# mjhoptics/ray-optics

Measured on AMD Instinct MI355X. Metric: ray-surface intersections/sec, higher is better.
Workload: dtype f64; 1 GPU; double-Gauss 13 interfaces (K=12), 1 field, 1 wvl, 1024x1024 pupil grid per GPU, FULL ray packets, device-generated rays (BASELINE.json configs[1]); interfaces=13, out_mode=FULL, field_index=0

## Files before the change

include/roxtrace.h:

```cpp
#ifndef ROXTRACE_H
#define ROXTRACE_H

#include <stddef.h>
#include <stdint.h>

#ifdef __cplusplus
extern "C" {
#endif
#if defined(__GNUC__) || defined(__clang__)
#pragma GCC visibility push(default)
#endif

#define ROX_ABI_VERSION 8
#define ROX_MAX_COEF 10
#define ROX_MAX_AP 4
#define ROX_SEG_DOUBLES 10

enum { ROX_TRANSMIT = 0, ROX_REFLECT = 1, ROX_DUMMY = 2, ROX_PHANTOM = 3 };
enum { ROX_SPHERICAL = 0, ROX_CONIC = 1, ROX_EVENPOLY = 2, ROX_RADIALPOLY = 3,
       ROX_YTOROID = 4, ROX_XTOROID = 5, ROX_THINLENS = 6 };
enum { ROX_PH_NONE = 0,
       ROX_PH_GRATING = 1,
       ROX_PH_DOE_RADIAL = 2,
       ROX_PH_HOLOGRAM = 3 };
// ... 90 lines not shown
    double cr_last_d[3];
    double d_cr_b4[3];
    double v_be;
    double image_pt[3];
} rox_wavefront;

typedef struct rox_opts {
    uint32_t flags;
    int32_t out_mode;
    int32_t first_surf;
    int32_t last_surf;
    double eps;
    double fuzz;
    double foc;
    double image_pt[2];
    rox_wavefront wf;
} rox_opts;

enum { ROX_FLD_EPD = 0, ROX_FLD_EPD_WIDE = 1, ROX_FLD_AIM_PT = 2, ROX_FLD_NA = 3,
       ROX_FLD_FNO = 4, ROX_FLD_AIM_DIR = 5 };

typedef struct rox_field {
    double pt0[3];
    double aim[2];
    double eprad;
    double z_enp;
    double vlx, vux, vly, vuy;
    double z_dir0;
    int32_t kind;
    int32_t rot_order;
    double rot[9];
    double cr_dir[2];
} rox_field;

typedef struct rox_grid {
    double start[2];
    double stop[2];
    int32_t num;
    int32_t kind;
    int32_t row_begin;
    int32_t row_count;
} rox_grid;

typedef struct rox_out {
    double *seg;
    double *op;
    uint8_t *status;
    int16_t *fail_surf;
    double *pupil;
    int64_t ld;
    int64_t *n_hits;
} rox_out;

typedef struct rox_system rox_system;

int rox_abi_version(void);
int rox_device_count(int *count);
int rox_set_device(int device);
const char *rox_last_error(void);

int rox_pin_host_memory(void *p, size_t bytes, void **device_ptr);
int rox_unpin_host_memory(void *p);
int rox_copy_async(void *dst, const void *src, size_t bytes, void *stream);
int rox_synchronize(void *stream);

int rox_system_create(const rox_surface *rows, int32_t n_ifcs,
                      const double *n_table, const double *wvls, int32_t n_wvls,
                      rox_system **out_sys);
int rox_system_destroy(rox_system *sys);
int rox_system_num_segments(const rox_system *sys, uint32_t flags,
                            int32_t *n_seg);

typedef struct rox_vig {
    rox_field fld;
    double start_dir[2];
    double unit_dir[2];
    int32_t xy;
    int32_t wvl_idx;
    int32_t stop_surf;
    int32_t max_iter;
} rox_vig;
int rox_calc_vignetting(rox_system *sys, int32_t n, const rox_vig *probs,
                        double eps, double *vig, int32_t *clip_surf, void *stream);

typedef struct rox_pupil_iter {
    rox_field fld;
    double start_r0;
    double r_target;
    int32_t xy;
    int32_t wvl_idx;
    int32_t indx;
    int32_t pad;
} rox_pupil_iter;
int rox_iterate_pupil_rays(rox_system *sys, int32_t n, const rox_pupil_iter *probs,
                           double eps, double *start_r, void *stream);

int rox_calc_psf(const double *opd, int32_t ndim, int32_t maxdim, double *psf,
                 uint32_t flags, void *stream);

int rox_trace_rays(rox_system *sys, int64_t n_rays,
                   const double *pt0, const double *dir0,
                   const int32_t *wvl_idx, int32_t wvl_idx_all,
                   const rox_opts *opts, const rox_out *out, void *stream);

int rox_trace_pupil_grid(rox_system *sys, const rox_field *fld,
                         const rox_grid *grid, int32_t wvl_idx,
// ... 274 lines not shown
```

include/roxtrace_diag.h:

```cpp
#ifndef ROXTRACE_DIAG_H
#define ROXTRACE_DIAG_H

#include "roxtrace.h"

#ifdef __cplusplus
extern "C" {
#endif
#if defined(__GNUC__) || defined(__clang__)
#pragma GCC visibility push(default)
#endif

int rox_time_pupil_grid(rox_system *sys, const rox_field *fld,
                        const rox_grid *grid, int32_t wvl_idx,
                        const rox_opts *opts, const rox_out *out,
                        void *stream, int32_t launches, double *mean_ms);

int rox_selftest_fp64(uint64_t n, uint64_t seed, uint64_t counts[4]);

int rox_diag_pack_launches(uint64_t counts[2]);

#if defined(__GNUC__) || defined(__clang__)
#pragma GCC visibility pop
#endif
#ifdef __cplusplus
}
#endif
#endif
```

ray-optics_amd/abi.py:

```python
import ctypes as C

ABI_VERSION = 8
MAX_COEF = 10
MAX_AP = 4
SEG_DOUBLES = 10

TRANSMIT, REFLECT, DUMMY, PHANTOM = 0, 1, 2, 3
MODE_NAMES = {'transmit': TRANSMIT, 'reflect': REFLECT, 'dummy': DUMMY,
              'phantom': PHANTOM}
SPHERICAL, CONIC, EVENPOLY, RADIALPOLY, YTOROID, XTOROID, THINLENS = 0, 1, 2, 3, 4, 5, 6
PROFILE_NAMES = {'Spherical': SPHERICAL, 'Conic': CONIC,
                 'EvenPolynomial': EVENPOLY, 'RadialPolynomial': RADIALPOLY,
                 'YToroid': YTOROID, 'XToroid': XTOROID}
PH_NONE, PH_GRATING, PH_DOE_RADIAL, PH_HOLOGRAM = 0, 1, 2, 3
AP_CIRCULAR, AP_RECTANGULAR, AP_ALWAYS_BLOCK = 0, 1, 2
OK, MISSED_SURFACE, TIR, BLOCKED, EVANESCENT = 0, 1, 2, 3, 4
OUT_FULL, OUT_LAST, OUT_HITS, OUT_OPD, OUT_HITS_COMPACT, OUT_FAN = 0, 1, 2, 3, 4, 5
CHECK_APERTURES = 1
INTERSECT_OBJ = 2
FILTER_PHANTOMS = 4
APPLY_VIGNETTING = 8
HOST_POINTERS = 16
HITS_APPEND = 32
FAST_FP64 = 64
# ... 206 lines not shown


WD_SLOT_COLS = 11
MAX_WD_AUX = 32
MAX_WD_COLS = 512


class Vig(C.Structure):
    _fields_ = [('fld', Field), ('start_dir', C.c_double * 2), ('unit_dir', C.c_double * 2),
                ('xy', C.c_int32), ('wvl_idx', C.c_int32), ('stop_surf', C.c_int32),
                ('max_iter', C.c_int32)]


class PupilIter(C.Structure):
    _fields_ = [('fld', Field), ('start_r0', C.c_double), ('r_target', C.c_double),
                ('xy', C.c_int32), ('wvl_idx', C.c_int32), ('indx', C.c_int32), ('pad', C.c_int32)]


assert C.sizeof(Aperture) == 40
assert C.sizeof(Vig) == 240
assert C.sizeof(Phase) == 168
assert C.sizeof(Surface) == 576
assert C.sizeof(Wavefront) == 512
assert C.sizeof(Opts) == 568
assert C.sizeof(Field) == 192
assert C.sizeof(Grid) == 48
assert C.sizeof(Out) == 56
assert C.sizeof(Aim) == 80
assert C.sizeof(Enp) == 136
assert C.sizeof(FocusPlane) == 544
assert C.sizeof(FocusStats) == 72
assert C.sizeof(FocusPsfStats) == 32
assert C.sizeof(ZernikeTerm) == 16
assert C.sizeof(ZernikeStats) == 56
assert C.sizeof(Footprint) == 144
assert C.sizeof(TxSurface) == 64
assert C.sizeof(TxItem) == 72
assert C.sizeof(SaItem) == 144
assert C.sizeof(SegFocus) == 136
assert C.sizeof(WmapItem) == 40
assert C.sizeof(WdItem) == 24

EXPORTS = ('rox_abi_version', 'rox_device_count', 'rox_set_device',
           'rox_last_error', 'rox_system_create', 'rox_system_destroy',
           'rox_system_num_segments', 'rox_trace_rays',
           'rox_trace_pupil_grid', 'rox_trace_pupil_grids', 'rox_trace_pupil_list',
           'rox_aim_chief_rays', 'rox_iterate_ray_raw', 'rox_find_real_enp', 'rox_calc_vignetting',
           'rox_iterate_pupil_rays', 'rox_calc_psf',
           'rox_pin_host_memory', 'rox_unpin_host_memory', 'rox_copy_async', 'rox_synchronize',
           'rox_spot_stats', 'rox_trace_through_focus', 'rox_trace_through_focus_grids',
           'rox_focus_psf', 'rox_focus_mtf', 'rox_focus_ee', 'rox_focus_gmtf', 'rox_focus_psf_ee',
           'rox_focus_zernike', 'rox_surface_footprints', 'rox_surface_transmission',
           'rox_surface_thinfilm', 'rox_projected_solid_angle', 'rox_segment_foci', 'rox_weighted_maps',
           'rox_wave_differentials')
DIAG_EXPORTS = ('rox_time_pupil_grid', 'rox_selftest_fp64', 'rox_diag_pack_launches')


def declare(lib):
    vp, i32, i64, dbl = C.c_void_p, C.c_int32, C.c_int64, C.c_double
    P = C.POINTER
    lib.rox_abi_version.restype = C.c_int
    lib.rox_abi_version.argtypes = []
    lib.rox_device_count.restype = C.c_int
    lib.rox_device_count.argtypes = [P(C.c_int)]
    lib.rox_set_device.restype = C.c_int
    lib.rox_set_device.argtypes = [C.c_int]
    lib.rox_last_error.restype = C.c_char_p
    lib.rox_last_error.argtypes = []
    lib.rox_system_create.restype = C.c_int
    lib.rox_system_create.argtypes = [P(Surface), i32, vp, vp, i32, P(vp)]
    lib.rox_system_destroy.restype = C.c_int
    lib.rox_system_destroy.argtypes = [vp]
    lib.rox_system_num_segments.restype = C.c_int
    lib.rox_system_num_segments.argtypes = [vp, C.c_uint32, P(i32)]
    lib.rox_trace_rays.restype = C.c_int
    lib.rox_trace_rays.argtypes = [vp, i64, vp, vp, vp, i32, P(Opts), P(Out), vp]
    lib.rox_trace_pupil_grid.restype = C.c_int
    lib.rox_trace_pupil_grid.argtypes = [vp, P(Field), P(Grid), i32, P(Opts),
                                         P(Out), vp]
    lib.rox_trace_pupil_grids.restype = C.c_int
    lib.rox_trace_pupil_grids.argtypes = [vp, i32, P(Field), P(i32), P(Grid), P(Opts),
                                          P(Out), vp]
    lib.rox_trace_pupil_list.restype = C.c_int
    lib.rox_trace_pupil_list.argtypes = [vp, P(Field), i64, vp, vp, i32,
                                         P(Opts), P(Out), vp]
    lib.rox_aim_chief_rays.restype = C.c_int
    lib.rox_aim_chief_rays.argtypes = [vp, i32, P(Aim), dbl, vp, vp, vp]
    lib.rox_iterate_ray_raw.restype = C.c_int
    lib.rox_iterate_ray_raw.argtypes = [vp, i32, P(Aim), dbl, vp, vp, vp, vp, vp]
    lib.rox_find_real_enp.restype = C.c_int
    lib.rox_find_real_enp.argtypes = [vp, i32, P(Enp), dbl, vp, vp, vp]
    lib.rox_calc_vignetting.restype = C.c_int
    lib.rox_calc_vignetting.argtypes = [vp, i32, P(Vig), dbl, vp, vp, vp]
    lib.rox_iterate_pupil_rays.restype = C.c_int
    lib.rox_iterate_pupil_rays.argtypes = [vp, i32, P(PupilIter), dbl, vp, vp]
    lib.rox_calc_psf.restype = C.c_int
    lib.rox_calc_psf.argtypes = [vp, i32, i32, vp, C.c_uint32, vp]
    lib.rox_pin_host_memory.restype = C.c_int
    lib.rox_pin_host_memory.argtypes = [vp, C.c_size_t, P(vp)]
    lib.rox_unpin_host_memory.restype = C.c_int
    lib.rox_unpin_host_memory.argtypes = [vp]
    lib.rox_copy_async.restype = C.c_int
    lib.rox_copy_async.argtypes = [vp, vp, C.c_size_t, vp]
    lib.rox_synchronize.restype = C.c_int
    lib.rox_synchronize.argtypes = [vp]
    lib.rox_spot_stats.restype = C.c_int
    lib.rox_spot_stats.argtypes = [vp, i64, vp, vp, i64, i32, vp, i32, vp, i32, P(SpotSummary), vp, vp]
    lib.rox_trace_through_focus.restype = C.c_int
    lib.rox_trace_through_focus.argtypes = [vp, P(Field), P(Grid), i32, P(Opts), i32, P(FocusPlane),
                                            vp, i64, vp, vp, vp]
    lib.rox_trace_through_focus_grids.restype = C.c_int
    lib.rox_trace_through_focus_grids.argtypes = [vp, i32, P(Field), P(i32), P(Grid), P(Opts), i32,
                                                  P(FocusPlane), vp, i64, vp, vp, vp]
    lib.rox_focus_psf.restype = C.c_int
    lib.rox_focus_psf.argtypes = [i32, i32, vp, i64, vp, vp, i32, i32, vp, vp, vp]
    lib.rox_focus_mtf.restype = C.c_int
    lib.rox_focus_mtf.argtypes = [i32, i32, vp, i32, vp, i32, vp, vp, vp]
    lib.rox_focus_ee.restype = C.c_int
    lib.rox_focus_ee.argtypes = [i32, i32, vp, i64, vp, i64, vp, i32, vp, vp, i32, vp, vp, vp, vp]
    lib.rox_focus_gmtf.restype = C.c_int
    lib.rox_focus_gmtf.argtypes = [i32, i32, vp, i64, vp, i64, i32, vp, i32, vp, vp, i32, vp, vp, vp, vp]
    lib.rox_focus_psf_ee.restype = C.c_int
    lib.rox_focus_psf_ee.argtypes = [i32, i32, vp, i32, vp, vp, i32, vp, vp, vp, vp]
    lib.rox_focus_zernike.restype = C.c_int
    lib.rox_focus_zernike.argtypes = [i32, i32, vp, i64, vp, P(Grid), vp, vp, i32, P(ZernikeTerm),
                                      vp, vp, vp]
    lib.rox_surface_footprints.restype = C.c_int
    lib.rox_surface_footprints.argtypes = [vp, C.c_uint32, C.c_uint32, i32, P(Out), i64, vp, vp, i32, vp, vp]
    lib.rox_surface_transmission.restype = C.c_int
    lib.rox_surface_transmission.argtypes = [vp, C.c_uint32, C.c_uint32, i32, P(Out), i64, vp, i32, vp, vp, vp, i64,
                                             vp, vp, vp]
    lib.rox_surface_thinfilm.restype = C.c_int
    lib.rox_surface_thinfilm.argtypes = [vp, C.c_uint32, C.c_uint32, i32, P(Out), i64, vp, vp, i32, vp, vp, vp, vp, vp,
                                         vp, vp, i64, vp, vp, vp]
    lib.rox_projected_solid_angle.restype = C.c_int
    lib.rox_projected_solid_angle.argtypes = [i32, i32, P(Out), i32, vp, i64, vp, vp, vp]
    lib.rox_segment_foci.restype = C.c_int
    lib.rox_segment_foci.argtypes = [vp, C.c_uint32, i32, P(Out), i64, vp, i64, vp, vp, vp]
    lib.rox_weighted_maps.restype = C.c_int
    lib.rox_weighted_maps.argtypes = [vp, C.c_uint32, i32, P(Out), i64, i32, vp, i64, vp, vp, i32, vp, i32, i32, vp, vp,
                                      vp, vp, vp]
    lib.rox_wave_differentials.restype = C.c_int
    lib.rox_wave_differentials.argtypes = [vp, C.c_uint32, i32, P(Out), i64, vp, i32, vp, i32, vp, i64, i64, vp, i64,
                                           vp, vp, vp, vp, vp]
    lib.rox_time_pupil_grid.restype = C.c_int
    lib.rox_time_pupil_grid.argtypes = [vp, P(Field), P(Grid), i32, P(Opts),
                                        P(Out), vp, i32, P(dbl)]
    lib.rox_selftest_fp64.restype = C.c_int
    lib.rox_selftest_fp64.argtypes = [C.c_uint64, C.c_uint64, P(C.c_uint64)]
    lib.rox_diag_pack_launches.restype = C.c_int
    lib.rox_diag_pack_launches.argtypes = [P(C.c_uint64)]
    return lib
```

ray-optics_amd/csrc/launch.hip:

```cpp
#include <atomic>
#include <climits>

#include "rox_system.hpp"
#include "../../include/roxtrace_diag.h"

namespace rox {

bool force_gtab()
{
    static const bool v = env_flag("ROX_FORCE_GTAB");
    return v;
}

static size_t launch_lds(const rox_system *s, int inst, bool per_ray_wvl, bool fast, bool gtab, int out_mode)
{
    const int feat = kInstances[inst];
    const bool phase = gtab || (feat & F_PHASE), aplist = gtab || (feat & F_APLIST);
    const bool global_table = gtab || gtab_of(feat, fast, out_mode) != 0;
    const size_t N = s->n_ifcs, Wn = per_ray_wvl ? (size_t)s->n_wvls : 1;
    size_t b = (global_table ? 0 : N * sizeof(dev_surface)) + Wn * N * sizeof(double) +
               ((phase && !global_table) ? Wn * N * kPhaseConsts * sizeof(double) : 0) +
               ((global_table && aplist) ? N * ROX_MAX_AP * sizeof(double) : 0) +
               ((size_t)s->n_wvls + N) * sizeof(double) + 2 * N * sizeof(int32_t);
    if (fast && !gtab)
// ... 42 lines not shown
        if (!(o->flags & ROX_HITS_APPEND) && out->ld < n_rays)
            return fail(ROX_E_ARG, "HITS_COMPACT: out.ld (%lld pairs of room) < n_rays (%lld)",
                        (long long)out->ld, (long long)n_rays);
        if (out->ld < 0)
            return fail(ROX_E_ARG, "HITS_COMPACT: negative out.ld");
    } else if (out->ld < n_rays) {
        return fail(ROX_E_ARG, "out.ld (%lld) < n_rays (%lld)", (long long)out->ld, (long long)n_rays);
    } else if (o->flags & ROX_HITS_APPEND) {
        return fail(ROX_E_ARG, "ROX_HITS_APPEND goes with ROX_OUT_HITS_COMPACT only");
    }
    if (!out->seg && n_rays > 0)
        return fail(ROX_E_ARG, "out.seg is null");
    if ((o->flags & ROX_FILTER_PHANTOMS) && sys->rows[0].mode == ROX_PHANTOM)
        return fail(ROX_E_UNSUPPORTED, "phantom object surface with filter_out_phantoms");
    return 0;
}

int check_field(const rox_field *fld)
{
    if (!fld)
        return fail(ROX_E_ARG, "null argument");
    if (fld->kind < ROX_FLD_EPD || fld->kind > ROX_FLD_AIM_DIR)
        return fail(ROX_E_ARG, "bad rox_field.kind %d", fld->kind);
    return 0;
}

int blocks_per_cu(int bs)
{
    static const int v = (int)env_int("ROX_BLOCKS_PER_CU", 0);
    return v > 0 ? v : 32 * 256 / bs;
}

int compact_blocks_per_cu()
{
    static const int v = (int)env_int("ROX_COMPACT_BLOCKS_PER_CU", 0);
    return v > 0 ? v : 1;
}

int32_t compact_small_want(const rox_system *sys, int64_t n_rays)
{
    static const int v = (int)env_int("ROX_COMPACT_SMALL_TILES", -1);
    if (v >= 0)
        return v;
    return n_rays <= (int64_t)sys->num_cus * kSmallTile ? sys->num_cus : 0;
}

int64_t rays_per_launch()
{
    static const int64_t v = [] {
        const long long n = env_int("ROX_RAYS_PER_LAUNCH", 0);
        return (n > 0 && n <= (1LL << 28)) ? (int64_t)n : (int64_t(1) << 28);
    }();
    return v;
}

static int pick_instance(int need)
{
    const int n = (int)(sizeof kInstances / sizeof kInstances[0]);
    static const int forced = (int)env_int("ROX_FORCE_INSTANCE", -1);
    if (forced >= 0 && forced < n && (need & ~kInstances[forced]) == 0)
        return forced;
    for (int i = 0; i < n; ++i)
        if ((need & ~kInstances[i]) == 0)
            return i;
    return n - 1;
}

constexpr int kSmallWavesPerCu = 24;
bool want_small(const rox_system *sys, int64_t total_rays, int out_mode, int feat, int64_t n_items)
{
    static const int forced = (int)env_int("ROX_SMALL_BLOCKS", -1);
    static const int per_cu_env = (int)env_int("ROX_SMALL_WAVES_PER_CU", 0);
    const int per_cu = per_cu_env > 0 ? per_cu_env : kSmallWavesPerCu;
    if (forced == 0 || forced == 1)
        return forced == 1;
    if (out_mode == ROX_OUT_FULL) {
        const int64_t big = block_of(ROX_OUT_FULL, feat, false);
        if (big <= ROX_BLOCK_SMALL)
            return false;
        if ((feat & kFeatNewton) && sys->n_newton * 4 > sys->n_ifcs - 1)
            return true;
        const int64_t per_item = (total_rays / n_items + big - 1) / big;
        const int64_t wgs = per_item * n_items, cus = sys->num_cus;
        const int64_t rounds = (wgs + cus - 1) / cus;
        const int64_t idle = rounds * cus - wgs;
        return rounds <= 4 && idle * 10 >= 3 * rounds * cus;
    }
    return (total_rays + 63) / 64 <= (int64_t)sys->num_cus * per_cu;
}

const TraceInstanceFns &trace_fns(int inst, const LaunchCfg &k)
{
#define ROX_TRACE_FNS(name, FEAT) &trace_##name,
#define ROX_TRACE_FAST_FNS(name, FEAT) &trace_##name##_fast,
    static const TraceInstanceFns *const fns[] = {ROX_TRACE_INSTANCES(ROX_TRACE_FNS)};
    static const TraceInstanceFns *const fast[] = {ROX_TRACE_INSTANCES(ROX_TRACE_FAST_FNS)};
#undef ROX_TRACE_FNS
#undef ROX_TRACE_FAST_FNS
    return k.gtab ? trace_general_gtab : *(k.fast ? fast : fns)[inst];
}

static int ensure_compact(StreamCtx *cx, int64_t tiles, hipStream_t st)
{
    CompactState &c = cx->compact;
    std::unique_lock<std::mutex> g(cx->ticket_mu);
    if (!c.d_ticket) {
// ... 39 lines not shown

int launch_setup(rox_system *sys, TraceArgs &a, int gen, bool prw, hipStream_t st, LaunchCfg &k,
                 int &inst)
{
    a.rows = sys->d_rows;
    a.n_table = sys->d_ntab;
    a.ph_consts = sys->d_phc;
    a.wvls = sys->d_wvls;
    a.slots = sys->d_slots[(a.opts.flags & ROX_FILTER_PHANTOMS) ? 1 : 0];
    a.n_ifcs = sys->n_ifcs;
    a.n_wvls = sys->n_wvls;
    int need = sys->features;
    if ((a.opts.flags & ROX_FILTER_PHANTOMS) && sys->n_seg[1] != sys->n_seg[0])
        need |= F_PHFILT;
    k.gen = gen;
    k.per_ray_wvl = prw;
    k.small = false;
    k.n_inline = 0;
    k.fast = use_fast(sys, a.opts);
    k.out_mode = a.opts.out_mode;
    k.stream = st;
    inst = pick_instance(need);
    k.gtab = false;
    k.lds = launch_lds(sys, inst, prw, k.fast, false, a.opts.out_mode);
    if (k.lds > kLdsLimit || force_gtab()) {
        inst = (int)(sizeof kInstances / sizeof kInstances[0]) - 1;
        k.fast = false;
        k.gtab = true;
        k.lds = launch_lds(sys, inst, prw, false, true, a.opts.out_mode);
        if (k.lds > kLdsLimit)
            return fail(ROX_E_UNSUPPORTED, "%d interfaces x %d wavelengths need %zu B of LDS for their "
                                           "indices and thresholds alone (max %zu)",
                        sys->n_ifcs, prw ? sys->n_wvls : 1, k.lds, kLdsLimit);
    }
    return 0;
}

int launch(rox_system *sys, TraceArgs &a, int gen, hipStream_t st)
{
    if (a.opts.out_mode == ROX_OUT_HITS_COMPACT && a.n_rays == 0) {
        if (!(a.opts.flags & ROX_HITS_APPEND))
            HIP_TRY(hipMemsetAsync(a.out.n_hits, 0, sizeof(int64_t), st));
        return 0;
    }
    if (a.n_rays == 0)
        return 0;
    const bool prw = a.wvl_idx != nullptr;
    LaunchCfg k;
    int inst;
    ROX_TRY(launch_setup(sys, a, gen, prw, st, k, inst));
    const int64_t total = a.n_rays;
    int64_t chunk_max = rays_per_launch();
    k.small = !prw && want_small(sys, total, a.opts.out_mode, kInstances[inst]);
    const bool compact = a.opts.out_mode == ROX_OUT_HITS_COMPACT;
    StreamCtx *cx = nullptr;
    bool two_pass = false;
    std::unique_lock<std::mutex> compact_lock;
    if (compact) {
        ROX_TRY(stream_ctx(sys, st, cx));
        compact_lock = std::unique_lock<std::mutex>(cx->compact_mu);
        const int tb = block_of(ROX_OUT_HITS_COMPACT, kInstances[inst]);
        two_pass = want_two_pass(total, a.out.seg);
        if (two_pass) {
            if (chunk_max > kTwoPassChunk)
                chunk_max = kTwoPassChunk;
            const int64_t per2 = total < chunk_max ? total : chunk_max;
            if (ensure_pack_scratch(cx, per2, a.out.status == nullptr) != 0) {
                (void)hipGetLastError();
                two_pass = false;
                chunk_max = rays_per_launch();
            }
        }
        const int64_t per = total < chunk_max ? total : chunk_max;
        a.small_tiles = two_pass ? 0 : compact_small_want(sys, per);
        ROX_TRY(ensure_compact(cx, two_pass ? (per + kPackTile - 1) / kPackTile
                                            : compact_tiles(per, a.small_tiles, tb), st));
    }
    const rox_out out0 = a.out;
    a.in_ld = total;
    const bool append = compact && (a.opts.flags & ROX_HITS_APPEND);
    if (append)
        HIP_TRY(hipMemcpyAsync(cx->compact.d_hits_base + 1, out0.n_hits, sizeof(int64_t), hipMemcpyDefault, st));
    int64_t n_launch = 0;
    for (int64_t base = 0; base < total; base += chunk_max, ++n_launch) {
        a.ray_base = base;
        a.n_rays = total - base < chunk_max ? total - base : chunk_max;
        if (compact) {
            a.tile_state = cx->compact.d_tiles;
            a.ticket = cx->compact.d_ticket;
            a.hits_base_in = (n_launch == 0 && !append) ? nullptr : cx->compact.d_hits_base + ((n_launch + 1) & 1);
            a.hits_total_out = (base + chunk_max >= total) ? out0.n_hits : cx->compact.d_hits_base + (n_launch & 1);
            a.epoch = ++cx->compact.epoch;
            a.out.status = out0.status ? out0.status + base : nullptr;
        } else {
            a.out.seg = out0.seg + base;
            a.out.op = out0.op ? out0.op + base : nullptr;
            a.out.status = out0.status ? out0.status + base : nullptr;
            a.out.fail_surf = out0.fail_surf ? out0.fail_surf + base : nullptr;
            a.out.pupil = out0.pupil ? out0.pupil + base : nullptr;
        }
        if (compact)
            (two_pass ? g_two_pass_launches : g_fused_pack_launches).fetch_add(1, std::memory_order_relaxed);
        if (two_pass) {
            TraceArgs h = a;
            h.opts.out_mode = ROX_OUT_HITS;
            h.opts.flags &= ~(uint32_t)ROX_HITS_APPEND;
            h.out.seg = cx->pack.d_xy;
            h.out.ld = cx->pack.cap;
            h.out.op = nullptr;
            h.out.fail_surf = nullptr;
            h.out.pupil = nullptr;
            h.out.n_hits = nullptr;
            h.out.status = out0.status ? out0.status + base : cx->pack.d_status;
            LaunchCfg kh = k;
            kh.out_mode = ROX_OUT_HITS;
            kh.lds = launch_lds(sys, inst, prw, kh.fast, k.gtab, ROX_OUT_HITS);
            const int hb = block_of(ROX_OUT_HITS, kInstances[inst], kh.small);
            int64_t hblocks = (a.n_rays + hb - 1) / hb;
            const int64_t hcap = (int64_t)sys->num_cus * blocks_per_cu(hb);
            kh.grid = dim3((unsigned)(hblocks > hcap ? hcap : hblocks));
            trace_fns(inst, kh).launch(kh, h);
            PackArgs p;
            p.status = h.out.status;
            p.xy = cx->pack.d_xy;
            p.ld = cx->pack.cap;
            p.n_rays = a.n_rays;
            p.tile_state = a.tile_state;
            p.ticket = a.ticket;
            p.hits_base_in = a.hits_base_in;
            p.hits_total_out = a.hits_total_out;
            p.epoch = a.epoch;
            p.dst = out0.seg;
            p.ld_dst = out0.ld;
            int64_t pblocks = (a.n_rays + kPackTile - 1) / kPackTile;
            const int64_t pcap = (int64_t)sys->num_cus * 2;
            launch_pack(p, (unsigned)(pblocks > pcap ? pcap : pblocks), st);
            continue;
        }
        const int bs = block_of(a.opts.out_mode, kInstances[inst], k.small);
        int64_t blocks = compact ? compact_tiles(a.n_rays, a.small_tiles, bs) : (a.n_rays + bs - 1) / bs;
        const int64_t cap = (int64_t)sys->num_cus * (compact ? compact_blocks_per_cu() : blocks_per_cu(bs));
        if (blocks > cap)
            blocks = cap;
        k.grid = dim3((unsigned)blocks);
        trace_fns(inst, k).launch(k, a);
    }
    a.n_rays = total;
    a.out = out0;
    HIP_TRY(hipGetLastError());
    return 0;
}

}

extern "C" int rox_diag_pack_launches(uint64_t counts[2])
{
    if (!counts)
        return rox::fail(ROX_E_ARG, "null argument");
    counts[0] = rox::g_fused_pack_launches.load();
    counts[1] = rox::g_two_pass_launches.load();
    return 0;
}
```

ray-optics_amd/csrc/rox_device.hpp:

```cpp
#pragma once
#include <hip/hip_runtime.h>

#include <cstddef>
#include <cstdint>
#include <cstring>
#include <type_traits>

#include "../../include/roxtrace.h"

#pragma clang fp contract(off)

#ifndef ROX_MIN_WAVES
#define ROX_MIN_WAVES 4
#endif
#ifndef ROX_STORE_NT
#define ROX_STORE_NT 1
#endif
#ifndef ROX_SLIM_FP64
#define ROX_SLIM_FP64 1
#endif
#ifndef ROX_IDENT_RT
#define ROX_IDENT_RT 1
#endif
#ifndef ROX_UNIT_FUSED
// ... 124 lines not shown
constexpr int F_POLY = F_EVEN | F_RADIAL | F_TOROID;
constexpr int F_ALL = F_POLY | F_APLIST | F_PHFILT | F_PHASE;
constexpr int F_GTAB = 128;
#ifndef ROX_GTAB_EXACT
#define ROX_GTAB_EXACT 1
#endif
#ifndef ROX_GTAB_FAST
#define ROX_GTAB_FAST 1
#endif
constexpr int gtab_of(int feat, bool fast, int out_mode)
{
    const int mask = fast ? ROX_GTAB_FAST : ROX_GTAB_EXACT;
    const bool newton = (feat & (1 | 2 | 4)) != 0;
    const int bit = (out_mode == ROX_OUT_FULL ? 4 : 1) << (newton ? 0 : 1);
    return ((feat & F_GTAB) || (mask & bit)) ? F_GTAB : 0;
}

struct v3 { double x, y, z; };
typedef double d2 __attribute__((ext_vector_type(2)));

typedef const double *tblp;
typedef const int32_t *tbli;
typedef const __attribute__((address_space(4))) double *ctblp;
typedef const __attribute__((address_space(4))) int32_t *ctbli;
typedef const __attribute__((address_space(4))) d2 *ctbl2;
__device__ __forceinline__ tbli ints_of(tblp p) { return reinterpret_cast<tbli>(p); }
__device__ __forceinline__ ctbli ints_of(ctblp p) { return (ctbli)p; }
__device__ __forceinline__ const d2 *pairs_of(tblp p) { return reinterpret_cast<const d2 *>(p); }
__device__ __forceinline__ ctbl2 pairs_of(ctblp p) { return (ctbl2)p; }

struct TraceArgs {
    const double *rows;
    const double *n_table;
    const double *ph_consts;
    const double *wvls;
    const int32_t *slots;
    int32_t n_ifcs, n_wvls;
    int64_t n_rays;
    int64_t ray_base;
    int64_t in_ld;
    const double *pt0, *dir0;
    const int32_t *wvl_idx;
    int32_t wvl_idx_all;
    const double *px, *py;
    int32_t axis_kind;
    int32_t axis_num;
    int32_t row_begin;
    uint64_t *tile_state;
    uint32_t *ticket;
    const int64_t *hits_base_in;
    int64_t *hits_total_out;
    uint32_t epoch;
    int32_t small_tiles;
    rox_field fld;
    rox_opts opts;
    rox_out out;
};

struct FocusArgs : TraceArgs {
    const rox_focus_plane *planes;
    int32_t n_planes;
    double *focus_rows;
    double *partial;
};

__device__ __forceinline__ double dot3(const v3 &a, const v3 &b)
{
    double acc = fma(a.x, b.x, 0.0);
    acc = fma(a.y, b.y, acc);
    return fma(a.z, b.z, acc);
}

template <class P>
__device__ __forceinline__ v3 rotate(P rt, int order, const v3 &v)
{
    v3 r;
    if (order == ROX_RT_C_ORDER) {
        r.x = fma(rt[2], v.z, fma(rt[0], v.x, fma(rt[1], v.y, 0.0)));
        r.y = fma(rt[5], v.z, fma(rt[3], v.x, fma(rt[4], v.y, 0.0)));
        r.z = fma(rt[8], v.z, fma(rt[6], v.x, fma(rt[7], v.y, 0.0)));
    } else {
        r.x = fma(rt[2], v.z, fma(rt[1], v.y, fma(rt[0], v.x, 0.0)));
        r.y = fma(rt[5], v.z, fma(rt[4], v.y, fma(rt[3], v.x, 0.0)));
        r.z = fma(rt[8], v.z, fma(rt[7], v.y, fma(rt[6], v.x, 0.0)));
    }
    return r;
}

__device__ __forceinline__ v3 cross3(const v3 &a, const v3 &b)
{
    return v3{a.y * b.z - a.z * b.y, a.z * b.x - a.x * b.z, a.x * b.y - a.y * b.x};
}

#ifndef ROX_WAVE_ALL_BALLOT
#define ROX_WAVE_ALL_BALLOT 1
#endif
__device__ __forceinline__ bool wave_all(bool p)
{
#if ROX_WAVE_ALL_BALLOT
    return __builtin_amdgcn_ballot_w64(!p) == 0;
#else
    return __all(p);
#endif
}

__device__ __forceinline__ bool in_band(double x)
// ... 1621 lines not shown
                const int first_pref = pmask ? __builtin_ctzll(pmask) : 64;
                const int take = first_pref < first_not ? first_pref + 1 : first_not;
                uint32_t v = lane < take ? (uint32_t)(w[k] & 0x3fffffffu) : 0u;
                for (int o = 32; o > 0; o >>= 1)
                    v += __shfl_xor(v, o);
                excl += v;
                if (first_pref < first_not) {
                    done = true;
                    break;
                }
                if (first_not < 64) {
                    consumed = k * 64 + first_not;
                    __builtin_amdgcn_s_sleep(1);
                    break;
                }
            }
            look -= consumed;
        }
        if (lane == 0)
            __hip_atomic_store(&st[tile], ts_pack(epoch, TS_PREFIX, excl + (uint32_t)total),
                               __ATOMIC_RELAXED, __HIP_MEMORY_SCOPE_AGENT);
    }
    return excl;
}

template <int kB, class ARGS>
__device__ __forceinline__ void finish_tile(ARGS &a, int64_t tile, int total,
                                            const d2 *stash, int64_t n_tiles, uint32_t *s_excl)
{
    const int lane = threadIdx.x & 63, wave = threadIdx.x >> 6;
    if (wave == 0) {
        const uint32_t excl = look_back(a.tile_state, a.epoch, tile, total, lane);
        if (lane == 0)
            *s_excl = excl;
    }
    __syncthreads();
    const uint32_t excl = (uint32_t)__builtin_amdgcn_readfirstlane((int)*s_excl);
    store_tile_pairs<kB>(reinterpret_cast<d2 *>(a.out.seg), a.out.ld, a.hits_base_in, (int64_t)excl,
                         total, stash, tile == n_tiles - 1 ? a.hits_total_out : nullptr);
}

constexpr int kSmallTile = 256;
__host__ __device__ inline int64_t compact_small_tiles(int64_t n_rays, int32_t want)
{
    const int64_t fit = n_rays / kSmallTile;
    return want < fit ? (want < 0 ? 0 : want) : fit;
}
__host__ __device__ inline int64_t compact_tiles(int64_t n_rays, int32_t want_small, int kB)
{
    const int64_t s = compact_small_tiles(n_rays, want_small);
    return s + (n_rays - s * kSmallTile + kB - 1) / kB;
}

struct FocusAcc {
    double n;
    double mx, my;
    double m2xy;
    double sr2;
    double mw, m2w;
    double wmin, wmax;
};
constexpr int kFocusStat = sizeof(FocusAcc) / sizeof(double);

__host__ __device__ inline FocusAcc focus_merge(const FocusAcc &a, const FocusAcc &b)
{
    if (b.n == 0)
        return a;
    if (a.n == 0)
        return b;
    FocusAcc r;
    r.n = a.n + b.n;
    const double f = b.n / r.n, g = a.n * b.n / r.n;
    const double dx = b.mx - a.mx, dy = b.my - a.my, dw = b.mw - a.mw;
    r.mx = a.mx + dx * f;
    r.my = a.my + dy * f;
    r.m2xy = (a.m2xy + b.m2xy) + (dx * dx + dy * dy) * g;
    r.sr2 = a.sr2 + b.sr2;
    r.mw = a.mw + dw * f;
    r.m2w = (a.m2w + b.m2w) + dw * dw * g;
    r.wmin = fmin(a.wmin, b.wmin);
    r.wmax = fmax(a.wmax, b.wmax);
    return r;
}

typedef const __attribute__((address_space(4))) rox_focus_plane *ConstPlanes;

__device__ __forceinline__ double wave_sum(double v)
{
#pragma unroll
    for (int o = 32; o > 0; o >>= 1)
        v += __shfl_xor(v, o);
    return v;
}

template <bool FAST, int kB, class ARGS>
__device__ __forceinline__ void focus_planes(ARGS &a, const RayEnd &e, const v3 &dir0, bool ok,
                                             uint32_t voff)
{
    const ConstPlanes planes = (ConstPlanes)a.planes;
    const int lane = threadIdx.x & 63, wave = threadIdx.x >> 6;
    const int64_t row_bytes = a.out.ld * 8;
    const double op = e.phs + e.opl;
    const double n_ok = (double)__popcll(__ballot(ok));
    for (int k = 0; k < a.n_planes; ++k) {
        const auto &pl = planes[k];
        double x = 0.0, y = 0.0, w = 0.0;
// ... 103 lines not shown
                    t = sqrt_le_threshold(ap[3] + a.opts.fuzz);
            }
            aplthr_w[i] = t;
        }
    __syncthreads();
    if ((FEAT & F_APLIST) && !kGtab) {
        stage_aperture_thresholds<FEAT>(tbl_w, N, a.opts.fuzz, threadIdx.x, kB);
        __syncthreads();
    }

    CtxT<TP> c;
    if constexpr (kGtab) {
        c.tbl = (ctblp)a.rows;
        c.phc = (ctblp)a.ph_consts + w0 * kPhaseConsts;
        c.aplthr = (FEAT & F_APLIST) ? aplthr_w : nullptr;
    } else {
        c.tbl = tbl_w;
        c.phc = phc_w;
        c.aplthr = nullptr;
    }
    c.ntab = ntab_w; c.wvls = wvls_w; c.apthr = apthr_w;
    c.slot = slot_w; c.nslots_before = slot_w + N;
    c.mu = mu_w;
    c.N = N;
    const uint32_t flags = a.opts.flags;
    c.check_ap = flags & ROX_CHECK_APERTURES;
    c.intersect_obj = flags & ROX_INTERSECT_OBJ;
    c.filter_ph = (FEAT & F_PHFILT) && (flags & ROX_FILTER_PHANTOMS);
    c.first_surf = a.opts.first_surf; c.last_surf = a.opts.last_surf;
    c.eps = a.opts.eps; c.fuzz = a.opts.fuzz;
    c.probe_surf = -1;
    const int64_t ld = a.out.ld;
    const int64_t n_small = kCompact ? compact_small_tiles(a.n_rays, a.small_tiles) : 0;
    const int64_t n_tiles = kCompact ? compact_tiles(a.n_rays, a.small_tiles, kB)
                          : (a.n_rays + kB - 1) / kB;

    __shared__ int64_t s_tile;
    __shared__ int32_t s_wcnt[kB / 64];
    __shared__ uint32_t s_excl;
    const int lane = threadIdx.x & 63, wave = threadIdx.x >> 6;
    constexpr bool kDefer = kCompact && ROX_COMPACT_DEFER;
    int64_t pend_tile = -1, pend_it = 0;
    int pend_total = 0;

    for (int64_t it = 0;; ++it) {
        int64_t tile;
        if (kCompact) {
            if (threadIdx.x == 0)
                s_tile = (int64_t)atomicAdd(&a.ticket[0], 1u);
            __syncthreads();
            tile = (int64_t)__builtin_amdgcn_readfirstlane((int)s_tile);
        } else {
            tile = (int64_t)blockIdx.x + it * gridDim.x;
        }
        if (tile >= n_tiles)
            break;
        int64_t r = tile * kB + threadIdx.x;
        bool active = r < a.n_rays;
        if (kCompact) {
            const bool small = tile < n_small;
            r = (small ? tile * kSmallTile : n_small * kSmallTile + (tile - n_small) * kB) + threadIdx.x;
            active = r < a.n_rays && (!small || threadIdx.x < kSmallTile);
        }
        RayEnd e;
        SegOut so;
        so.base = reinterpret_cast<char *>(a.out.seg);
        so.row_bytes = ld * 8;
        so.voff = (uint32_t)r * 8u;
        v3 pt0{0, 0, 0}, dir0{0, 0, 1};
        int wi = a.wvl_idx_all;
        bool wi_ok = true;
        if (active) {
            const int64_t rg = a.ray_base + r;
            if (GEN == GEN_PUPIL) {
                double px, py;
                if (a.axis_kind == AXIS_PRODUCT) {
                    px = a.px[a.row_begin + rg / a.axis_num];
                    py = a.py[rg % a.axis_num];
                } else {
                    px = a.px[rg];
                    py = a.py[rg];
                }
                ray_start(a.fld, flags, px, py, pt0, dir0);
                if (!kCompact && a.out.pupil) {
                    a.out.pupil[r] = px;
                    a.out.pupil[ld + r] = py;
                }
            } else {
                pt0 = v3{a.pt0[rg], a.pt0[a.in_ld + rg], a.pt0[2 * a.in_ld + rg]};
                dir0 = v3{a.dir0[rg], a.dir0[a.in_ld + rg], a.dir0[2 * a.in_ld + rg]};
            }
            if (PER_RAY_WVL) {
                wi = a.wvl_idx[rg];
                wi_ok = (wi >= 0 && wi < a.n_wvls);
                if (!wi_ok)
                    wi = 0;
            }
        }
        if constexpr (kFast)
            trace_ray_fast<kTrace, PER_RAY_WVL, FEAT>(c, so, pt0, dir0, wi, active, e);
        else if constexpr (ROX_REDUCED_STRAIGHT && OUT_MODE != ROX_OUT_FULL)
            trace_ray_reduced<kTrace, PER_RAY_WVL, FEAT>(c, pt0, dir0, wi, active, e);
        else
            trace_ray<kTrace, PER_RAY_WVL, FEAT>(c, so, pt0, dir0, wi, active, e);
        if (active) {
            if (PER_RAY_WVL && !wi_ok) {
// ... 338 lines not shown
```

ray-optics_amd/csrc/rox_system.hpp:

```cpp
#pragma once

#include <mutex>
#include <vector>

#include "rox_device.hpp"
#include "rox_host.hpp"

namespace rox {

constexpr char kHipWhere[] = "";
inline int (&fail)(int code, const char *fmt, ...) = host_fail;


struct AxesCache {
    double *d = nullptr;
    int32_t cap = 0;
    double key[4] = {0, 0, 0, 0};
    int32_t num = 0;
};

struct CompactState {
    uint64_t *d_tiles = nullptr;
    int64_t tiles_cap = 0;
    uint32_t *d_ticket = nullptr;
// ... 33 lines not shown
    std::vector<double> prm;
    int32_t num = 0;
};

struct StreamCtx {
    hipStream_t stream = nullptr;
    AxesCache axes;
    CompactState compact;
    PackScratch pack;
    StageArena stage;
    BatchItems batch;
    FocusBlock focus;
    std::mutex enqueue_mu;
    std::mutex batch_mu;
    std::mutex stage_mu;
    std::mutex compact_mu;
    std::mutex ticket_mu;
};

}

struct rox_system {
    int device = 0;
    int32_t n_ifcs = 0, n_wvls = 0;
    std::vector<rox_surface> rows;
    double *d_rows = nullptr;
    double *d_ntab = nullptr;
    double *d_phc = nullptr;
    double *d_wvls = nullptr;
    int32_t *d_slots[2] = {nullptr, nullptr};
    int32_t n_seg[2] = {0, 0};
    int num_cus = 256;
    int features = 0;
    int n_newton = 0;
    std::mutex mu;
    std::vector<rox::StreamCtx *> ctxs;
    char *h_search = nullptr;
    size_t h_search_cap = 0;
    std::mutex search_mu;
};

namespace rox {

int stream_ctx(rox_system *sys, hipStream_t st, StreamCtx *&cx);
std::unique_lock<std::mutex> enqueue_lock(rox_system *sys, hipStream_t st);

constexpr size_t kLdsLimit = 160 * 1024 - 64;
bool force_gtab();
int64_t rays_per_launch();
int blocks_per_cu(int bs);
int compact_blocks_per_cu();
int32_t compact_small_want(const rox_system *sys, int64_t n_rays);
bool want_small(const rox_system *sys, int64_t total_rays, int out_mode, int feat, int64_t n_items = 1);
int check_opts(const rox_system *sys, const rox_opts *o, const rox_out *out, int64_t n_rays);
int check_field(const rox_field *fld);
const TraceInstanceFns &trace_fns(int inst, const LaunchCfg &k);
int launch_setup(rox_system *sys, TraceArgs &a, int gen, bool prw, hipStream_t st, LaunchCfg &k, int &inst);
int launch(rox_system *sys, TraceArgs &a, int gen, hipStream_t st);

int grid_args(rox_system *sys, const rox_field *fld, const rox_grid *grid, int32_t wvl_idx,
              const rox_opts *opts, const rox_out *out, TraceArgs &a);

}
```

ray-optics_amd/csrc/trace_entries.hip:

```cpp
#include <algorithm>
#include <cstring>

#include "rox_system.hpp"
#include "../../include/roxtrace_diag.h"

#pragma clang fp contract(off)

using namespace rox;

namespace {

__global__ void pupil_axes_kernel(double x0, double y0, double sx, double sy, int num,
                                  double *px, double *py)
{
    if (threadIdx.x > 1)
        return;
    double v = threadIdx.x == 0 ? x0 : y0;
    const double step = threadIdx.x == 0 ? sx : sy;
    double *out = threadIdx.x == 0 ? px : py;
    for (int k = 0; k < num; ++k) {
        out[k] = v;
        v += step;
    }
}
// ... 228 lines not shown
    auto enq = enqueue_lock(sys, st);
    ROX_TRY(prepare_grid(sys, fld, grid, wvl_idx, opts, out, st, a));
    if (!(opts->flags & ROX_HOST_POINTERS))
        return launch(sys, a, GEN_PUPIL, st);
    ROX_TRY(stage(s, sys, st, opts, out, a.n_rays));
    return launch_staged(s, sys, a, GEN_PUPIL, st);
}

int rox_trace_pupil_grids(rox_system *sys, int32_t n_grids, const rox_field *flds,
                          const int32_t *wvl_idx, const rox_grid *grid, const rox_opts *opts,
                          const rox_out *outs, void *stream)
{
    if (!sys)
        return fail(ROX_E_ARG, "null system");
    if (n_grids < 0 || (n_grids > 0 && (!flds || !wvl_idx || !opts || !outs)))
        return fail(ROX_E_ARG, "null argument");
    if (n_grids == 0)
        return 0;
    hipStream_t st = (hipStream_t)stream;
    for (int32_t i = 0; i < n_grids; ++i) {
        if (opts[i].flags & (ROX_HOST_POINTERS | ROX_HITS_APPEND))
            return fail(ROX_E_UNSUPPORTED, "rox_trace_pupil_grids: device pointers only, no ROX_HITS_APPEND "
                                           "(item %d)", i);
        if (opts[i].out_mode != opts[0].out_mode ||
            ((opts[i].flags ^ opts[0].flags) & (ROX_FILTER_PHANTOMS | ROX_FAST_FP64)))
            return fail(ROX_E_ARG, "rox_trace_pupil_grids: out_mode, ROX_FILTER_PHANTOMS and ROX_FAST_FP64 "
                                   "must be the same for every item (item %d)", i);
    }
    auto enq = enqueue_lock(sys, st);
    std::vector<TraceArgs> items((size_t)n_grids);
    for (int32_t i = 0; i < n_grids; ++i)
        ROX_TRY(prepare_grid(sys, &flds[i], grid, wvl_idx[i], &opts[i], &outs[i], st, items[i]));
    const int64_t R = items[0].n_rays;
    const bool compact = opts[0].out_mode == ROX_OUT_HITS_COMPACT;
    if (n_grids == 1 || n_grids > 65535 || R > rays_per_launch() || R == 0) {
        for (int32_t i = 0; i < n_grids; ++i)
            ROX_TRY(launch(sys, items[i], GEN_PUPIL, st));
        return 0;
    }
    LaunchCfg k;
    int inst = 0;
    for (int32_t i = 0; i < n_grids; ++i) {
        ROX_TRY(launch_setup(sys, items[i], GEN_PUPIL, false, st, k, inst));
        items[i].in_ld = R;
        items[i].ray_base = 0;
    }
    StreamCtx *cx;
    ROX_TRY(stream_ctx(sys, st, cx));
    std::lock_guard<std::mutex> lock(cx->batch_mu);
    BatchItems &b = cx->batch;
    k.small = want_small(sys, (int64_t)n_grids * R, opts[0].out_mode, kInstances[inst], n_grids);
    const int bs = block_of(opts[0].out_mode, kInstances[inst], k.small);
    int64_t blocks = (R + bs - 1) / bs;
    if (compact) {
        if ((int64_t)n_grids > b.tickets_cap)
            HIP_TRY(regrow_zeroed(b.d_tickets, b.tickets_cap, n_grids,
                                  sizeof(uint32_t) * 2 * (size_t)n_grids, st));
        const int32_t small = ((int64_t)n_grids * R <= (int64_t)sys->num_cus * kSmallTile)
                                  ? compact_small_want(sys, R) : 0;
        const int64_t tiles = compact_tiles(R, small, bs);
        blocks = tiles;
        if ((int64_t)n_grids * tiles > b.tiles_cap) {
            HIP_TRY(regrow_zeroed(b.d_tiles, b.tiles_cap, n_grids * tiles,
                                  sizeof(uint64_t) * (size_t)(n_grids * tiles), st));
            b.epoch = 0;
        }
        ++b.epoch;
        for (int32_t i = 0; i < n_grids; ++i) {
            items[i].small_tiles = small;
            items[i].tile_state = b.d_tiles + (size_t)i * tiles;
            items[i].ticket = b.d_tickets + 2 * (size_t)i;
            items[i].hits_base_in = nullptr;
            items[i].hits_total_out = outs[i].n_hits;
            items[i].epoch = b.epoch;
        }
    }
    const int64_t cap = (int64_t)sys->num_cus * (compact ? compact_blocks_per_cu() : blocks_per_cu(bs));
    if (blocks > cap)
        blocks = cap;
    k.grid = dim3((unsigned)blocks, (unsigned)n_grids);
    static const bool no_inline = env_flag("ROX_BATCH_NO_INLINE");
    if (n_grids <= kInlineItems && !no_inline) {
        k.n_inline = n_grids;
        trace_fns(inst, k).batch(k, items.data());
        HIP_TRY(hipGetLastError());
        return 0;
    }
    if (n_grids > b.cap) {
        const int32_t want = n_grids < 64 ? 64 : n_grids;
        HIP_TRY(release(b.d_items, b.cap));
        HIP_TRY(regrow(b.h_items, b.cap, want,
                       sizeof(TraceArgs) * (size_t)want * BatchItems::kSlots, hipHostMallocDefault));
        HIP_TRY(regrow(b.d_items, b.cap, want, sizeof(TraceArgs) * (size_t)want));
        b.last.clear();
        for (bool &live : b.ev_live)
            live = false;
    }
    const size_t items_bytes = sizeof(TraceArgs) * (size_t)n_grids;
    static const bool always_upload = env_flag("ROX_BATCH_ALWAYS_UPLOAD");
    const bool same_items = !always_upload && b.last.size() == items_bytes &&
                            memcmp(b.last.data(), items.data(), items_bytes) == 0;
    if (!same_items) {
        const uint32_t slot = b.slot++ % BatchItems::kSlots;
        if (!b.ev[slot])
            HIP_TRY(hipEventCreateWithFlags(&b.ev[slot], hipEventDisableTiming));
        if (b.ev_live[slot])
// ... 83 lines not shown
```

ray-optics_amd/engine.py:

```python
import collections
import ctypes as C
import functools
import os
import threading

import numpy as np

from . import abi
from .table import SurfaceTable

_HERE = os.path.dirname(os.path.abspath(__file__))
LIB_PATH = os.environ.get('ROX_LIB') or os.path.join(_HERE, 'libroxtrace.so')
_lib = None


class EngineError(RuntimeError):
    pass


def load_library():
    global _lib
    if _lib is None:
        import torch
        if not os.environ.get('ROX_LIB'):
# ... 133 lines not shown


SEG_FOCUS_DTYPE = np.dtype([(name, np.int64) for name in ('n', 'n_flat', 'n_bad', 'n_in')] +
                           [('w_sum', np.float64), ('w_in', np.float64), ('a_mean', np.float64, (2,)),
                            ('b_mean', np.float64, (2,))] +
                           [(name, np.float64) for name in ('m_aa', 'm_ab', 'm_bb', 'z_in_min', 'z_in_max',
                                                            'z_out_min', 'z_out_max')])
assert SEG_FOCUS_DTYPE.itemsize == C.sizeof(abi.SegFocus)

WMAP_ITEM_DTYPE = np.dtype([(name, np.int64) for name in ('n_in', 'n_out', 'n_bad', 'q_in', 'q_out')])
WD_ITEM_DTYPE = np.dtype([(name, np.int64) for name in ('n', 'n_bad', 'pivot_ray')])
assert WD_ITEM_DTYPE.itemsize == C.sizeof(abi.WdItem)
assert WMAP_ITEM_DTYPE.itemsize == C.sizeof(abi.WmapItem)


def seg_focus_derive(rec):
    with np.errstate(divide='ignore', invalid='ignore'):
        maa, mab, mbb, w = rec['m_aa'], rec['m_ab'], rec['m_bb'], rec['w_sum']
        conv = mbb > 0
        zeta = np.where(conv, -mab / np.where(conv, mbb, 1.0), np.nan)
        ms_0 = maa / w
        ms_min = np.where(conv, np.maximum(maa - mab * mab / np.where(conv, mbb, 1.0), 0.0) / w, ms_0)
        lo = np.minimum(rec['z_in_min'], rec['z_out_min'])
        hi = np.maximum(rec['z_in_max'], rec['z_out_max'])
        inside = conv & (zeta >= lo) & (zeta <= hi)
    return zeta, ms_min, ms_0, inside


ZERNIKE_STATS_DTYPE = np.dtype([('n', np.int64), ('n_outside', np.int64), ('rms', np.float64),
                                ('rms_residual', np.float64), ('pv_residual', np.float64),
                                ('cond', np.float64), ('fit', np.int32), ('reserved', np.int32)])
assert ZERNIKE_STATS_DTYPE.itemsize == C.sizeof(abi.ZernikeStats)


def zernike_stats_view(raw):
    return records_view(raw, ZERNIKE_STATS_DTYPE)


class FocusRows:

    def __init__(self, rows, status):
        self.rows = rows
        self.status = status

    def to_host(self):
        return self.rows.cpu().numpy(), self.status.cpu().numpy()


def _f64(x, shape):
    return np.ascontiguousarray(np.broadcast_to(np.asarray(x, dtype=np.float64), shape))


def padded_ld(R):
    if R <= 0:
        return 1
    return (R + 511) // 512 * 512 + 256


def _default_pool_budget():
    env = os.environ.get('ROX_PINNED_POOL_MB')
    if env:
        return int(env) << 20
    try:
        ram = os.sysconf('SC_PAGE_SIZE') * os.sysconf('SC_PHYS_PAGES')
    except (ValueError, OSError, AttributeError):
        ram = 32 << 30
    return int(min(4 << 30, max(256 << 20, ram // 8)))


class PinnedPool:

    def __init__(self):
        self._lock = threading.Lock()
        self._returned = collections.deque()
        self._free = {}
        self._shelved = 0
        self.budget = _default_pool_budget()

    @property
    def _held(self):
        with self._lock:
            self._drain()
            return self._shelved

    @staticmethod
    def _round(nbytes):
        if nbytes > (64 << 20):
            return (nbytes + (16 << 20) - 1) // (16 << 20) * (16 << 20)
        n = 4096
        while n < nbytes:
            n *= 2
        return n

    def take(self, torch, nbytes):
        n = self._round(max(int(nbytes), 1))
        with self._lock:
            self._drain()
            lst = self._free.get(n)
            t = None
            if lst:
                t = lst.pop()
                self._shelved -= n
        if t is None:
            t = torch.empty(n, dtype=torch.uint8).pin_memory()
        return _Lease(self, n, t)

    def give_back(self, n, t):
        self._returned.append((n, t))

# ... 1252 lines not shown
```

Baseline: 59.63 billion ray-surface intersections/s.

## Remap FULL-mode tiles so each XCD writes contiguous spans; cap packet padding

In FULL output mode, the tile index each workgroup processes is permuted so that consecutive tiles within a span of 8*group are assigned to the same XCD, based on round-robin dispatch across the 8 XCDs. The intent is to make each XCD's writes to the strided ray-packet arrays contiguous, improving L2 and memory locality. The packet leading dimension moves into a library function that caps padding relative to the ray count. A diagnostic export exposes the tile map. This risks mismatching the real dispatch order and changes output stride for small ray counts.

```diff
diff --git a/include/roxtrace.h b/include/roxtrace.h
--- a/include/roxtrace.h
+++ b/include/roxtrace.h
@@ -166,6 +166,8 @@
     int64_t *n_hits;
 } rox_out;
 
+int64_t rox_packet_ld(int64_t n_rays);
+
 typedef struct rox_system rox_system;
 
 int rox_abi_version(void);
diff --git a/include/roxtrace_diag.h b/include/roxtrace_diag.h
--- a/include/roxtrace_diag.h
+++ b/include/roxtrace_diag.h
@@ -19,6 +19,9 @@
 
 int rox_diag_pack_launches(uint64_t counts[2]);
 
+int rox_diag_full_tile_map(int64_t n_tiles, int32_t group, int64_t grid, int32_t wg0,
+                           int64_t *tiles);
+
 #if defined(__GNUC__) || defined(__clang__)
 #pragma GCC visibility pop
 #endif
diff --git a/ray-optics_amd/abi.py b/ray-optics_amd/abi.py
--- a/ray-optics_amd/abi.py
+++ b/ray-optics_amd/abi.py
@@ -282,8 +282,9 @@
            'rox_focus_psf', 'rox_focus_mtf', 'rox_focus_ee', 'rox_focus_gmtf', 'rox_focus_psf_ee',
            'rox_focus_zernike', 'rox_surface_footprints', 'rox_surface_transmission',
            'rox_surface_thinfilm', 'rox_projected_solid_angle', 'rox_segment_foci', 'rox_weighted_maps',
-           'rox_wave_differentials')
-DIAG_EXPORTS = ('rox_time_pupil_grid', 'rox_selftest_fp64', 'rox_diag_pack_launches')
+           'rox_wave_differentials', 'rox_packet_ld')
+DIAG_EXPORTS = ('rox_time_pupil_grid', 'rox_selftest_fp64', 'rox_diag_pack_launches',
+                'rox_diag_full_tile_map')
 
 
 def declare(lib):
@@ -373,6 +374,8 @@
     lib.rox_wave_differentials.restype = C.c_int
     lib.rox_wave_differentials.argtypes = [vp, C.c_uint32, i32, P(Out), i64, vp, i32, vp, i32, vp, i64, i64, vp, i64,
                                            vp, vp, vp, vp, vp]
+    lib.rox_packet_ld.restype = i64
+    lib.rox_packet_ld.argtypes = [i64]
     lib.rox_time_pupil_grid.restype = C.c_int
     lib.rox_time_pupil_grid.argtypes = [vp, P(Field), P(Grid), i32, P(Opts),
                                         P(Out), vp, i32, P(dbl)]
@@ -380,4 +383,6 @@
     lib.rox_selftest_fp64.argtypes = [C.c_uint64, C.c_uint64, P(C.c_uint64)]
     lib.rox_diag_pack_launches.restype = C.c_int
     lib.rox_diag_pack_launches.argtypes = [P(C.c_uint64)]
+    lib.rox_diag_full_tile_map.restype = C.c_int
+    lib.rox_diag_full_tile_map.argtypes = [i64, i32, i64, i32, P(i64)]
     return lib
diff --git a/ray-optics_amd/csrc/launch.hip b/ray-optics_amd/csrc/launch.hip
--- a/ray-optics_amd/csrc/launch.hip
+++ b/ray-optics_amd/csrc/launch.hip
@@ -118,6 +118,15 @@
         return (n > 0 && n <= (1LL << 28)) ? (int64_t)n : (int64_t(1) << 28);
     }();
     return v;
+}
+
+constexpr int32_t kFullTileGroup = 32;
+int32_t full_tile_group(bool small)
+{
+    static const long long env = env_int("ROX_FULL_TILE_GROUP", -1);
+    if (env >= 0)
+        return (int32_t)(env > kMaxTileGroup ? kMaxTileGroup : env);
+    return small ? 0 : kFullTileGroup;
 }
 
 static int pick_instance(int need)
@@ -263,6 +272,7 @@
     const int64_t total = a.n_rays;
     int64_t chunk_max = rays_per_launch();
     k.small = !prw && want_small(sys, total, a.opts.out_mode, kInstances[inst]);
+    a.tile_group = a.opts.out_mode == ROX_OUT_FULL ? full_tile_group(k.small) : 0;
     const bool compact = a.opts.out_mode == ROX_OUT_HITS_COMPACT;
     StreamCtx *cx = nullptr;
     bool two_pass = false;
@@ -364,6 +374,28 @@
 
 }
 
+extern "C" int64_t rox_packet_ld(int64_t n_rays)
+{
+    constexpr int64_t kPadDoubles = 256;
+    if (n_rays <= 0)
+        return 1;
+    const int64_t cap = n_rays / 16 > 256 ? n_rays / 16 : 256;
+    const int64_t want = (n_rays + 511) / 512 * 512 + kPadDoubles;
+    return want - n_rays <= cap ? want : (n_rays + cap) / 8 * 8;
+}
+
+extern "C" int rox_diag_full_tile_map(int64_t n_tiles, int32_t group, int64_t grid, int32_t wg0,
+                                      int64_t *tiles)
+{
+    if (n_tiles < 0 || n_tiles > INT32_MAX || group < 0 || group > rox::kMaxTileGroup || grid < 1 ||
+        wg0 < 0 || (n_tiles > 0 && !tiles))
+        return rox::fail(ROX_E_ARG, "rox_diag_full_tile_map: bad argument");
+    for (int64_t wg = 0; wg < grid; ++wg)
+        for (int64_t t = wg; t < n_tiles; t += grid)
+            tiles[t] = rox::full_tile_map(t, n_tiles, group, (uint32_t)wg0 % rox::kXcds);
+    return 0;
+}
+
 extern "C" int rox_diag_pack_launches(uint64_t counts[2])
 {
     if (!counts)
diff --git a/ray-optics_amd/csrc/rox_device.hpp b/ray-optics_amd/csrc/rox_device.hpp
--- a/ray-optics_amd/csrc/rox_device.hpp
+++ b/ray-optics_amd/csrc/rox_device.hpp
@@ -200,6 +200,7 @@
     int64_t *hits_total_out;
     uint32_t epoch;
     int32_t small_tiles;
+    int32_t tile_group;
     rox_field fld;
     rox_opts opts;
     rox_out out;
@@ -1927,6 +1928,20 @@
     return s + (n_rays - s * kSmallTile + kB - 1) / kB;
 }
 
+constexpr int kXcds = 8;
+constexpr int32_t kMaxTileGroup = 1 << 16;
+__host__ __device__ constexpr int64_t full_tile_map(int64_t t, int64_t n_tiles, int32_t group, uint32_t wg0)
+{
+    if (group <= 0)
+        return t;
+    const uint32_t span = (uint32_t)kXcds * (uint32_t)group;
+    const uint32_t start = (uint32_t)t / span * span;
+    if ((int64_t)start + span > n_tiles)
+        return t;
+    const uint32_t j = (uint32_t)t - start;
+    return (int64_t)(start + (j + wg0) % kXcds * (uint32_t)group + j / kXcds);
+}
+
 struct FocusAcc {
     double n;
     double mx, my;
@@ -2136,6 +2151,8 @@
             tile = (int64_t)__builtin_amdgcn_readfirstlane((int)s_tile);
         } else {
             tile = (int64_t)blockIdx.x + it * gridDim.x;
+            if constexpr (OUT_MODE == ROX_OUT_FULL)
+                tile = full_tile_map(tile, n_tiles, a.tile_group, blockIdx.y * gridDim.x % kXcds);
         }
         if (tile >= n_tiles)
             break;
diff --git a/ray-optics_amd/csrc/rox_system.hpp b/ray-optics_amd/csrc/rox_system.hpp
--- a/ray-optics_amd/csrc/rox_system.hpp
+++ b/ray-optics_amd/csrc/rox_system.hpp
@@ -109,6 +109,7 @@
 int compact_blocks_per_cu();
 int32_t compact_small_want(const rox_system *sys, int64_t n_rays);
 bool want_small(const rox_system *sys, int64_t total_rays, int out_mode, int feat, int64_t n_items = 1);
+int32_t full_tile_group(bool small);
 int check_opts(const rox_system *sys, const rox_opts *o, const rox_out *out, int64_t n_rays);
 int check_field(const rox_field *fld);
 const TraceInstanceFns &trace_fns(int inst, const LaunchCfg &k);
diff --git a/ray-optics_amd/csrc/trace_entries.hip b/ray-optics_amd/csrc/trace_entries.hip
--- a/ray-optics_amd/csrc/trace_entries.hip
+++ b/ray-optics_amd/csrc/trace_entries.hip
@@ -304,6 +304,9 @@
     k.small = want_small(sys, (int64_t)n_grids * R, opts[0].out_mode, kInstances[inst], n_grids);
     const int bs = block_of(opts[0].out_mode, kInstances[inst], k.small);
     int64_t blocks = (R + bs - 1) / bs;
+    if (opts[0].out_mode == ROX_OUT_FULL)
+        for (int32_t i = 0; i < n_grids; ++i)
+            items[i].tile_group = full_tile_group(k.small);
     if (compact) {
         if ((int64_t)n_grids > b.tickets_cap)
             HIP_TRY(regrow_zeroed(b.d_tickets, b.tickets_cap, n_grids,
diff --git a/ray-optics_amd/engine.py b/ray-optics_amd/engine.py
--- a/ray-optics_amd/engine.py
+++ b/ray-optics_amd/engine.py
@@ -209,9 +209,7 @@
 
 
 def padded_ld(R):
-    if R <= 0:
-        return 1
-    return (R + 511) // 512 * 512 + 256
+    return int(load_library().rox_packet_ld(int(R)))
 
 
 def _default_pool_budget():
```

Result: faster. 61.69 billion ray-surface intersections/s, median of 6 (+3.4%).
